# chengstone/cchess-zero

Measured on NVIDIA H100. Metric: mcts_node_expansions_per_sec, higher is better.
Workload: dtype fp16

## Files before the change

### cchess_zero_b200/_lib.py

```python
import ctypes as C
import os

_HERE = os.path.dirname(os.path.abspath(__file__))
LIB_PATH = os.path.join(_HERE, "libcchess_b200.so")

NSQ, NLABEL, MAXCHILD, ENC_LEN, STATUS_BYTES, MT_WORDS = 90, 2086, 128, 1260, 112, 626
F32, BF16, F16, BOARD = 0, 1, 2, 3
ERR_NAMES = {1: "NOMOVES", 2: "NOLABEL", 4: "DEPTH", 8: "ARENA", 16: "CHILDREN"}

_lib = None


class EngineError(RuntimeError):
    pass


def _sig(L):
    vp, i32, i64 = C.c_void_p, C.c_int, C.c_int64
    L.cz_last_error.restype = C.c_char_p
    L.cz_labels.argtypes = [vp]
    L.cz_label_index.argtypes = [i32, i32]
    L.cz_unflipped_index.argtypes = [vp]
    L.cz_from_state.argtypes = [C.c_char_p, vp]
    L.cz_to_state.argtypes = [vp, C.c_char_p]
# ... 21 lines not shown
    L.cz_engine_leaf_hashes.argtypes = [vp, vp]
    L.cz_engine_root_keys.argtypes = [vp, vp, vp]
    L.cz_engine_play_status.argtypes = [vp, vp, vp, vp]
    L.cz_engine_status_packed.argtypes = [vp, vp, vp]
    L.cz_engine_unfinished.argtypes = [vp, vp, vp]
    L.cz_engine_unfinished_async.argtypes = [vp, vp, vp]
    L.cz_engine_root_children.argtypes = [vp, vp, vp, vp, vp, vp, vp, vp]
    L.cz_engine_play.argtypes = [vp, vp, vp]
    L.cz_engine_status.argtypes = [vp, vp, vp, vp, vp, vp, vp, vp]
    L.cz_engine_counters.argtypes = [vp, vp, vp]
    L.cz_engine_tree_signature.argtypes = [vp, vp, i32, vp, i64, vp]
    L.cz_net_first_conv.argtypes = [vp, i32, vp, vp, vp, vp]
    L.cz_net_first_conv_tc.argtypes = [vp, i32, vp, vp, vp, vp]
    L.cz_net_first_conv_mma.argtypes = [vp, i32, vp, vp, vp]
    L.cz_net_heads.argtypes = [vp, i32, vp, vp, vp, vp, vp, vp, vp, vp, vp, vp, vp, vp, vp]
    L.cz_host_choose_moves.argtypes = [i32, vp, vp, vp, i32, vp, vp, vp, vp, i32]
    L.cz_net_heads_tc.argtypes = [vp, i32, vp, vp, vp, vp, vp, vp, vp, vp, vp, vp, vp, vp, vp]
    L.cz_net_heads_fc.argtypes = [vp, vp, i32, vp, vp, vp, vp, vp, vp, vp, vp, vp]
    L.cz_net_split_tf32.argtypes = [vp, vp, vp, i64, vp]
    L.cz_net_epilogue_split.argtypes = [vp, vp, vp, vp, vp, vp, vp, i64, vp]
    L.cz_net_tower_blob_bytes.argtypes = [i32]
    L.cz_net_tower_blob_bytes.restype = i64
    L.cz_net_tower_small.argtypes = [vp, i32, i32, i32, vp, vp, vp, vp, vp, vp, vp, vp]


def lib():
    global _lib
    if _lib is None:
        from . import build as _build

        distributed = "RANK" in os.environ or os.environ.get("CCHESS_NO_REBUILD", "0") == "1"
        if not (distributed and os.path.exists(LIB_PATH)):
            try:
                _build.build()
            except Exception as e:
                if not os.path.exists(LIB_PATH):
                    raise EngineError("libcchess_b200.so is missing and could not be built: %s" % e)
        L = C.CDLL(LIB_PATH)
        _sig(L)
        _lib = L
    return _lib


def check(rc, what=""):
    if rc != 0:
        raise EngineError("%s failed (%d): %s" % (what or "cchess_b200 call", rc, lib().cz_last_error().decode()))
# ... 1 lines not shown
```

### cchess_zero_b200/csrc/cz_net.cu

```cuda
#include <cuda_fp16.h>
#include <cuda_runtime.h>
#include <stdint.h>
#include <stdlib.h>
#include <string.h>

#include "../../include/cchess_b200.h"
#include "cz_wgmma.cuh"

namespace {

using namespace cz_sm90;

__global__ void __launch_bounds__(256) k_first_conv(const uint8_t *__restrict__ boards, int B, const __half *__restrict__ w ,
                                                     const float4 *__restrict__ bias , __half *__restrict__ out ) {
    __shared__ uint8_t pb[11 * 12 + 12];
    const int pos = blockIdx.x;
    const uint8_t *bd = boards + (size_t)pos * 96;
    if (threadIdx.x < 132) {
        const int r = threadIdx.x / 12 - 1, f = threadIdx.x % 12 - 1;
        pb[threadIdx.x] = (r >= 0 && r < 9 && f >= 0 && f < 10) ? bd[r * 9 + f] : (uint8_t)0;
    }
    __syncthreads();
    const int hw = threadIdx.x >> 4, l16 = threadIdx.x & 15;
    const float4 b0 = bias[l16 * 2], b1 = bias[l16 * 2 + 1];
// ... 3 lines not shown
        int pc[9];
#pragma unroll
        for (int t = 0; t < 9; t++) pc[t] = c0[(t / 3) * 12 + (t % 3)];
        float acc[8] = {b0.x, b0.y, b0.z, b0.w, b1.x, b1.y, b1.z, b1.w};
#pragma unroll
        for (int t = 0; t < 9; t++) {
            if (pc[t]) {
                const uint4 raw = __ldg(reinterpret_cast<const uint4 *>(w + ((size_t)(t * 14 + pc[t] - 1) * 128 + l16 * 8)));
                const __half2 *h2 = reinterpret_cast<const __half2 *>(&raw);
#pragma unroll
                for (int k = 0; k < 4; k++) {
                    const float2 v = __half22float2(h2[k]);
                    acc[2 * k] += v.x;
                    acc[2 * k + 1] += v.y;
                }
            }
        }
        uint4 o;
        __half2 *oh = reinterpret_cast<__half2 *>(&o);
#pragma unroll
        for (int k = 0; k < 4; k++) oh[k] = __floats2half2_rn(fmaxf(acc[2 * k], 0.f), fmaxf(acc[2 * k + 1], 0.f));
        *reinterpret_cast<uint4 *>(out + ((size_t)pos * 90 + cell) * 128 + l16 * 8) = o;
    }
}

__device__ __forceinline__ void mma16816(float (&c)[4], const uint32_t (&a)[4], const uint32_t (&b)[2]) {
    asm volatile("mma.sync.aligned.m16n8k16.row.col.f32.f16.f16.f32 {%0,%1,%2,%3}, {%4,%5,%6,%7}, {%8,%9}, {%0,%1,%2,%3};\n"
                 : "+f"(c[0]), "+f"(c[1]), "+f"(c[2]), "+f"(c[3])
                 : "r"(a[0]), "r"(a[1]), "r"(a[2]), "r"(a[3]), "r"(b[0]), "r"(b[1]));
}

constexpr int FCM_POS = 4;
__global__ void __launch_bounds__(256) k_first_conv_mma(const uint8_t *__restrict__ boards, int B, const uint2 *__restrict__ wfrag ,
                                                         __half *__restrict__ out ) {
    __shared__ uint2 sW[9 * 16 * 32];
    __shared__ uint8_t pb[FCM_POS][11 * 12 + 12];
    const int tid = threadIdx.x, warp = tid >> 5, lane = tid & 31, g = lane >> 2, t = lane & 3;
    const int pos0 = blockIdx.x * FCM_POS;
    for (int i = tid; i < 9 * 16 * 32 / 2; i += 256) reinterpret_cast<uint4 *>(sW)[i] = __ldg(reinterpret_cast<const uint4 *>(wfrag) + i);
    for (int i = tid; i < FCM_POS * 144; i += 256) {
        const int p = i / 144, j = i - p * 144;
        uint8_t v = 0;
        if (j < 132 && pos0 + p < B) {
            const int r = j / 12 - 1, f = j % 12 - 1;
            if (r >= 0 && r < 9 && f >= 0 && f < 10) v = boards[(size_t)(pos0 + p) * 96 + r * 9 + f];
        }
        pb[p][j] = v;
    }
    __syncthreads();
#pragma unroll 1
    for (int tile = warp; tile < FCM_POS * 6; tile += 8) {
        const int p = tile / 6, mt = tile - p * 6;
// ... 499 lines not shown
    if (cudaGetLastError() != cudaSuccess) return CZ_ECUDA;
    if (cudaEventRecord(ev_join[dev], side[dev]) != cudaSuccess) return CZ_ECUDA;
    dim3 grid((B + 63) / 64, NPAD / 64);
    k_policy_fc<<<grid, 128, smem, st>>>((const __half *)hp, B, (const __half *)wp, bp, logits);
    if (cudaGetLastError() != cudaSuccess) return CZ_ECUDA;
    if (cudaStreamWaitEvent(st, ev_join[dev], 0) != cudaSuccess) return CZ_ECUDA;
    return CZ_OK;
}

int cz_net_heads(const void *x, int B, const float *wh, const float *bh, const float *w1t, const float *b1, const float *w2, const float *b2,
                 const void *wp, const float *bp, void *hp_scratch, float *hv_scratch, float *logits, float *value, void *stream) {
    if (!x || !wh || !bh || !hp_scratch || !hv_scratch || B <= 0) return CZ_EINVAL;
    static const bool legacy = getenv("CCHESS_HEAD_CONV") && !strcmp(getenv("CCHESS_HEAD_CONV"), "simt");
    if (legacy) k_head_conv<<<B, 256, 0, (cudaStream_t)stream>>>((const __half *)x, B, wh, bh, (__half *)hp_scratch, hv_scratch);
    else k_head_conv_mma<false><<<B, 192, 0, (cudaStream_t)stream>>>((const __half *)x, B, wh, bh, (__half *)hp_scratch, hv_scratch);
    if (cudaGetLastError() != cudaSuccess) return CZ_ECUDA;
    return cz_net_heads_fc(hp_scratch, hv_scratch, B, w1t, b1, w2, b2, wp, bp, logits, value, stream);
}


int cz_net_heads_tc(const void *x, int B, const float *wh, const float *bh, const float *w1t, const float *b1, const float *w2, const float *b2,
                    const void *wp_tiled, const float *bp, void *hp_tiled_scratch, float *hv_scratch, float *logits, float *value, void *stream) {
    if (!x || !wh || !bh || !w1t || !b1 || !w2 || !b2 || !wp_tiled || !bp || !hp_tiled_scratch || !hv_scratch || !logits || !value || B <= 0) return CZ_EINVAL;
    cudaStream_t st = (cudaStream_t)stream;
    const int smem = 2 * FC_TILE_BYTES;
    if (cudaFuncSetAttribute(k_policy_fc_tc, cudaFuncAttributeMaxDynamicSharedMemorySize, smem) != cudaSuccess) return CZ_ECUDA;
    k_head_conv_mma<true><<<B, 192, 0, st>>>((const __half *)x, B, wh, bh, (__half *)hp_tiled_scratch, hv_scratch);
    if (cudaGetLastError() != cudaSuccess) return CZ_ECUDA;
    int dev = 0;
    if (cudaGetDevice(&dev) != cudaSuccess || dev < 0 || dev >= 64) return CZ_ECUDA;
    static cudaStream_t side[64] = {nullptr};
    static cudaEvent_t ev_fork[64] = {nullptr}, ev_join[64] = {nullptr};
    if (!side[dev]) {
        if (cudaStreamCreateWithFlags(&side[dev], cudaStreamNonBlocking) != cudaSuccess) return CZ_ECUDA;
        if (cudaEventCreateWithFlags(&ev_fork[dev], cudaEventDisableTiming) != cudaSuccess) return CZ_ECUDA;
        if (cudaEventCreateWithFlags(&ev_join[dev], cudaEventDisableTiming) != cudaSuccess) return CZ_ECUDA;
    }
    if (cudaEventRecord(ev_fork[dev], st) != cudaSuccess) return CZ_ECUDA;
    if (cudaStreamWaitEvent(side[dev], ev_fork[dev], 0) != cudaSuccess) return CZ_ECUDA;
    k_value_mlp<<<(B + VM_POS - 1) / VM_POS, 256, 0, side[dev]>>>(hv_scratch, B, w1t, b1, w2, b2, value);
    if (cudaGetLastError() != cudaSuccess) return CZ_ECUDA;
    if (cudaEventRecord(ev_join[dev], side[dev]) != cudaSuccess) return CZ_ECUDA;
    dim3 grid((B + 127) / 128, 17);
    k_policy_fc_tc<<<grid, 256, smem, st>>>((const uint4 *)hp_tiled_scratch, B, (const uint4 *)wp_tiled, bp, logits);
    if (cudaGetLastError() != cudaSuccess) return CZ_ECUDA;
    if (cudaStreamWaitEvent(st, ev_join[dev], 0) != cudaSuccess) return CZ_ECUDA;
    return CZ_OK;
}

int cz_net_split_tf32(const float *y, float *hi, void *x2, long long n_pix, void *stream) {
    if (!y || !hi || !x2 || n_pix <= 0) return CZ_EINVAL;
    const long long n8 = n_pix * 16;
    int dev = 0, sms = 132;
    if (cudaGetDevice(&dev) == cudaSuccess) cudaDeviceGetAttribute(&sms, cudaDevAttrMultiProcessorCount, dev);
    long long blocks = (n8 + 255) / 256;
    if (blocks > 8LL * sms) blocks = 8LL * sms;
    k_split_tf32<<<(unsigned)blocks, 256, 0, (cudaStream_t)stream>>>(reinterpret_cast<const float4 *>(y), reinterpret_cast<float4 *>(hi),
                                                                    reinterpret_cast<uint4 *>(x2), n8);
    return cudaGetLastError() == cudaSuccess ? CZ_OK : CZ_ECUDA;
}

int cz_net_epilogue_split(const float *t, const void *s, const float *bias, const float *skip, float *x, float *hi, void *x2, long long n_pix, void *stream) {
    if (!t || !bias || n_pix <= 0 || (!x && !hi) || ((hi == nullptr) != (x2 == nullptr))) return CZ_EINVAL;
    const long long n8 = n_pix * 16;
    int dev = 0, sms = 132;
    if (cudaGetDevice(&dev) == cudaSuccess) cudaDeviceGetAttribute(&sms, cudaDevAttrMultiProcessorCount, dev);
    long long blocks = (n8 + 255) / 256;
// ... 10 lines not shown
```

### cchess_zero_b200/csrc/cz_tower.cu

```cuda
#include <cuda.h>
#include <cuda_fp16.h>
#include <cuda_runtime.h>
#include <stdint.h>
#include <stdio.h>
#include <stdlib.h>
#include <string.h>

#include "../../include/cchess_b200.h"
#include "cz_wgmma.cuh"

namespace {

using namespace cz_sm90;

constexpr int ROWS = 152;
constexpr int P0 = 12;
constexpr int LBO_A = ROWS * 16;
constexpr int A_BYTES = 16 * LBO_A;
constexpr int NMATH = 256;
constexpr int NMATH_WARPS = NMATH / 32;
constexpr int NTHREADS = NMATH + 32;

__device__ __forceinline__ uint32_t img_off(int chunk, int row) { return (uint32_t)(chunk * LBO_A + row * 16); }

// ... 256 lines not shown
                float s0 = a.bh[0], s1 = a.bh[1], s2 = a.bh[2];
#pragma unroll 4
                for (int c8 = 0; c8 < 16; c8++) {
                    const uint4 raw = *reinterpret_cast<const uint4 *>(bufX + img_off(c8, P0 + j));
                    const __half2 *h2 = reinterpret_cast<const __half2 *>(&raw);
#pragma unroll
                    for (int k = 0; k < 4; k++) {
                        const float2 x = __half22float2(h2[k]);
                        const int c = c8 * 8 + 2 * k;
                        s0 += x.x * __ldg(a.wh + c) + x.y * __ldg(a.wh + c + 1);
                        s1 += x.x * __ldg(a.wh + 128 + c) + x.y * __ldg(a.wh + 128 + c + 1);
                        s2 += x.x * __ldg(a.wh + 256 + c) + x.y * __ldg(a.wh + 256 + c + 1);
                    }
                }
                const int ci = rr * 10 + ff;
                *reinterpret_cast<__half2 *>(a.hp + (size_t)pos * 192 + ci * 2) = __floats2half2_rn(fmaxf(s0, 0.f), fmaxf(s1, 0.f));
                a.hv[(size_t)pos * 96 + ci] = fmaxf(s2, 0.f);
            }
            if (rank == 0 && tid < 12) a.hp[(size_t)pos * 192 + 180 + tid] = __float2half(0.f);
        }
    }
    __syncthreads();
    if (CL > 1) cluster_sync_all();
}

typedef CUresult (*EncodeTiledFn)(CUtensorMap *, CUtensorMapDataType, cuuint32_t, void *, const cuuint64_t *, const cuuint64_t *, const cuuint32_t *,
                                  const cuuint32_t *, CUtensorMapInterleave, CUtensorMapSwizzle, CUtensorMapL2promotion, CUtensorMapFloatOOBfill);

EncodeTiledFn encode_tiled() {
    static EncodeTiledFn fn = nullptr;
    if (!fn) {
        void *p = nullptr;
        cudaDriverEntryPointQueryResult q;
        if (cudaGetDriverEntryPoint("cuTensorMapEncodeTiled", &p, cudaEnableDefault, &q) != cudaSuccess || q != cudaDriverEntryPointSuccess) return nullptr;
        fn = (EncodeTiledFn)p;
    }
    return fn;
}

template <int CL, bool ASYNC_ST>
int launch_tower(const CUtensorMap &map, const TowerArgs &a, cudaStream_t st) {
    constexpr int NC = 128 / CL, S = CL == 1 ? 4 : (CL == 2 ? 8 : 16);
    const int n_layers = 1 + a.n_conv;
    const size_t smem = 2 * (size_t)A_BYTES + (size_t)S * NC * 256 + (size_t)n_layers * NC * 4;
    if (cudaFuncSetAttribute(k_tower_small<CL, ASYNC_ST>, cudaFuncAttributeMaxDynamicSharedMemorySize, (int)smem) != cudaSuccess) return CZ_ECUDA;
    cudaLaunchConfig_t cfg = {};
// ... 44 lines not shown
    struct TraceDump {
        const TowerArgs &a; cudaStream_t st; long long *dev; int *calls;
        ~TraceDump() {
            if (!a.trace || ++*calls != 20) return;
            long long h[64 * 8];
            cudaStreamSynchronize(st);
            cudaMemcpy(h, dev, sizeof(h), cudaMemcpyDeviceToHost);
            fprintf(stderr, "tower trace (clock64 deltas): layer: in_ready->w_ready, ->mma_issued, ->mma_done, ->(same), ->stores_issued, ->next in_ready\n");
            for (int L = 0; L < a.n_conv; L++) {
                const long long *r = h + L * 8, nxt = L + 1 < a.n_conv ? h[(L + 1) * 8] : r[5];
                fprintf(stderr, "  L%02d: %6lld %6lld %6lld %6lld %6lld %6lld | layer %6lld\n", L, r[1] - r[0], r[2] - r[1], r[3] - r[2], r[4] - r[3], r[5] - r[4], nxt - r[5], nxt - r[0]);
            }
        }
    } dump{a, st, trace_dev, &trace_calls};
    static const bool generic_st = getenv("CCHESS_TOWER_ST") && !strcmp(getenv("CCHESS_TOWER_ST"), "generic");
    switch (cluster) {
        case 1: return generic_st ? launch_tower<1, false>(map, a, st) : launch_tower<1, true>(map, a, st);
        case 2: return generic_st ? launch_tower<2, false>(map, a, st) : launch_tower<2, true>(map, a, st);
        case 4: return generic_st ? launch_tower<4, false>(map, a, st) : launch_tower<4, true>(map, a, st);
        default: return generic_st ? launch_tower<8, false>(map, a, st) : launch_tower<8, true>(map, a, st);
    }
}

}
```

### cchess_zero_b200/csrc/cz_wgmma.cuh

```cuda
#pragma once
#include <stdint.h>

namespace cz_sm90 {

__device__ __forceinline__ uint32_t smem_u32(const void *p) { return (uint32_t)__cvta_generic_to_shared(p); }

__device__ __forceinline__ uint64_t gmma_desc(uint32_t smem_addr, uint32_t lbo_bytes) {
    return (uint64_t)((smem_addr >> 4) & 0x3FFFu) | ((uint64_t)((lbo_bytes >> 4) & 0x3FFFu) << 16) | ((uint64_t)(128u >> 4) << 32);
}

__device__ __forceinline__ void wgmma_fence() { asm volatile("wgmma.fence.sync.aligned;" ::: "memory"); }
__device__ __forceinline__ void wgmma_commit() { asm volatile("wgmma.commit_group.sync.aligned;" ::: "memory"); }
template <int N>
__device__ __forceinline__ void wgmma_wait() { asm volatile("wgmma.wait_group.sync.aligned %0;" ::"n"(N) : "memory"); }

template <int R>
__device__ __forceinline__ void fence_regs(float (&d)[R]) {
#pragma unroll
    for (int i = 0; i < R; i++) asm volatile("" : "+f"(d[i])::"memory");
}

template <int N>
struct Wgmma;
template <> struct Wgmma<16> {
    static __device__ __forceinline__ void mma(float (&d)[8], uint64_t da, uint64_t db, uint32_t scale_d) {
        asm volatile("{\n\t.reg .pred p;\n\tsetp.ne.b32 p, %10, 0;\n\t"
                     "wgmma.mma_async.sync.aligned.m64n16k16.f32.f16.f16 {"
                     "%0, %1, %2, %3, %4, %5, %6, %7"
                     "}, %8, %9, p, 1, 1, 0, 0;\n\t}"
                     : "+f"(d[0]), "+f"(d[1]), "+f"(d[2]), "+f"(d[3]), "+f"(d[4]), "+f"(d[5]), "+f"(d[6]), "+f"(d[7])
                     : "l"(da), "l"(db), "r"(scale_d));
    }
};
template <> struct Wgmma<32> {
    static __device__ __forceinline__ void mma(float (&d)[16], uint64_t da, uint64_t db, uint32_t scale_d) {
        asm volatile("{\n\t.reg .pred p;\n\tsetp.ne.b32 p, %18, 0;\n\t"
                     "wgmma.mma_async.sync.aligned.m64n32k16.f32.f16.f16 {"
                     "%0, %1, %2, %3, %4, %5, %6, %7, %8, %9, %10, %11, %12, %13, %14, %15"
                     "}, %16, %17, p, 1, 1, 0, 0;\n\t}"
                     : "+f"(d[0]), "+f"(d[1]), "+f"(d[2]), "+f"(d[3]), "+f"(d[4]), "+f"(d[5]), "+f"(d[6]), "+f"(d[7]),
                       "+f"(d[8]), "+f"(d[9]), "+f"(d[10]), "+f"(d[11]), "+f"(d[12]), "+f"(d[13]), "+f"(d[14]), "+f"(d[15])
                     : "l"(da), "l"(db), "r"(scale_d));
// ... 14 lines not shown
    }
};
template <> struct Wgmma<128> {
    static __device__ __forceinline__ void mma(float (&d)[64], uint64_t da, uint64_t db, uint32_t scale_d) {
        asm volatile("{\n\t.reg .pred p;\n\tsetp.ne.b32 p, %66, 0;\n\t"
                     "wgmma.mma_async.sync.aligned.m64n128k16.f32.f16.f16 {"
                     "%0, %1, %2, %3, %4, %5, %6, %7, %8, %9, %10, %11, %12, %13, %14, %15, "
                     "%16, %17, %18, %19, %20, %21, %22, %23, %24, %25, %26, %27, %28, %29, %30, %31, "
                     "%32, %33, %34, %35, %36, %37, %38, %39, %40, %41, %42, %43, %44, %45, %46, %47, "
                     "%48, %49, %50, %51, %52, %53, %54, %55, %56, %57, %58, %59, %60, %61, %62, %63"
                     "}, %64, %65, p, 1, 1, 0, 0;\n\t}"
                     : "+f"(d[0]), "+f"(d[1]), "+f"(d[2]), "+f"(d[3]), "+f"(d[4]), "+f"(d[5]), "+f"(d[6]), "+f"(d[7]),
                       "+f"(d[8]), "+f"(d[9]), "+f"(d[10]), "+f"(d[11]), "+f"(d[12]), "+f"(d[13]), "+f"(d[14]), "+f"(d[15]),
                       "+f"(d[16]), "+f"(d[17]), "+f"(d[18]), "+f"(d[19]), "+f"(d[20]), "+f"(d[21]), "+f"(d[22]), "+f"(d[23]),
                       "+f"(d[24]), "+f"(d[25]), "+f"(d[26]), "+f"(d[27]), "+f"(d[28]), "+f"(d[29]), "+f"(d[30]), "+f"(d[31]),
                       "+f"(d[32]), "+f"(d[33]), "+f"(d[34]), "+f"(d[35]), "+f"(d[36]), "+f"(d[37]), "+f"(d[38]), "+f"(d[39]),
                       "+f"(d[40]), "+f"(d[41]), "+f"(d[42]), "+f"(d[43]), "+f"(d[44]), "+f"(d[45]), "+f"(d[46]), "+f"(d[47]),
                       "+f"(d[48]), "+f"(d[49]), "+f"(d[50]), "+f"(d[51]), "+f"(d[52]), "+f"(d[53]), "+f"(d[54]), "+f"(d[55]),
                       "+f"(d[56]), "+f"(d[57]), "+f"(d[58]), "+f"(d[59]), "+f"(d[60]), "+f"(d[61]), "+f"(d[62]), "+f"(d[63])
                     : "l"(da), "l"(db), "r"(scale_d));
    }
};

}
```

### cchess_zero_b200/net.py

```python
import os

import numpy as np
import torch
import torch.nn as nn
import torch.nn.functional as F

NLABEL = 2086


class RefBatchNorm(nn.Module):

    def __init__(self, ch, eps=1e-5, decay=0.999, update_moving_stats=False):
        super().__init__()
        self.eps, self.decay, self.update = eps, decay, update_moving_stats
        self.register_buffer("running_mean", torch.zeros(ch))
        self.register_buffer("running_var", torch.ones(ch))

    def forward(self, x):
        if self.training:
            mean = x.mean(dim=(0, 2, 3))
            var = x.var(dim=(0, 2, 3), unbiased=False)
            if self.update:
                n = x.numel() / x.shape[1]
                with torch.no_grad():
# ... 420 lines not shown
            return True
        return False

    def make_input(self, B):
        return torch.zeros((B, 96), dtype=torch.uint8, device=self.hp.device)

    @torch.no_grad()
    def __call__(self, boards, logits_out, value_out):
        B = boards.shape[0]
        assert B <= self.max_batch and boards.dtype == torch.uint8 and logits_out.dtype == torch.float32
        assert self.blob.numel() * 2 == self._lib.cz_net_tower_blob_bytes(self.n_conv)
        st = self._C.c_void_p(torch.cuda.current_stream().cuda_stream)
        rc = self._lib.cz_net_tower_small(boards.data_ptr(), B, self.cluster, self.n_conv, self.w1.data_ptr(), self.blob.data_ptr(), self.bias.data_ptr(),
                                          self.wh.data_ptr(), self.bh.data_ptr(), self.hp.data_ptr(), self.hv.data_ptr(), st)
        if rc:
            raise RuntimeError("cz_net_tower_small failed (%d)" % rc)
        rc = self._lib.cz_net_heads_fc(self.hp.data_ptr(), self.hv.data_ptr(), B, self.w1t.data_ptr(), self.bv1.data_ptr(), self.w2.data_ptr(),
                                       self.b2t.data_ptr(), self.wp.data_ptr(), self.bp.data_ptr(), logits_out.data_ptr(), value_out.data_ptr(), st)
        if rc:
            raise RuntimeError("cz_net_heads_fc failed (%d)" % rc)
        return None


class _Tf32:
    def __init__(self, on):
        self.on = on

    def __enter__(self):
        self.prev = (torch.backends.cudnn.allow_tf32, torch.backends.cuda.matmul.allow_tf32)
        torch.backends.cudnn.allow_tf32 = self.on
        torch.backends.cuda.matmul.allow_tf32 = self.on

    def __exit__(self, *a):
        torch.backends.cudnn.allow_tf32, torch.backends.cuda.matmul.allow_tf32 = self.prev


def train_step_module(net, opt, x, pi, z, learning_rate, c_l2=1e-4, global_norm=100, group=None):
    import torch.distributed as dist
    net.train()
    for gp in opt.param_groups:
        gp["lr"] = float(learning_rate)
    logits, value = net(x)
    policy_loss = (-(pi * F.log_softmax(logits, dim=1)).sum(dim=1)).mean()
    value_loss = F.mse_loss(value, z)
    l2 = sum((p * p).sum() for p in net.parameters()) * (0.5 * c_l2)
    loss = value_loss + policy_loss + l2
# ... 31 lines not shown
        self.c_l2 = 0.0001
        self.momentum = 0.9
        self.global_norm = 100
        self.global_step = 0
        self.precision = precision or os.environ.get("CCHESS_NN_PRECISION", "fp16")
        if seed is not None:
            torch.manual_seed(seed)
        self.net = PolicyValueNet(res_block_nums, self.filters_size, update_moving_stats).to(self.device)
        self.net = self.net.to(memory_format=torch.channels_last)
        self.opt = torch.optim.SGD(self.net.parameters(), lr=1e-3, momentum=self.momentum, nesterov=True)
        self._plan = None
        self.weights_version = 0
        self.train_restore()

    def plan(self):
        if self._plan is None:
            self.net.eval()
            self._plan = make_plan(self.net, self.precision, owner=self)
        self._plan.refresh_if_stale()
        return self._plan

    def native_plan(self, max_batch, first_conv=None):
        self.net.eval()
        return NativePlan(self.net, max_batch, first_conv, owner=self)

    def small_plan(self, max_batch, cluster=None):
        self.net.eval()
        return SmallTowerPlan(self.net, max_batch, cluster, owner=self)

    @property
    def nn_dtype(self):
        return _DT[self.precision]

    def forward_device(self, nn_in, logits_out=None, value_out=None):
        return self.plan()(nn_in, logits_out, value_out)

    def forward(self, positions):
        x = torch.as_tensor(np.asarray(positions, dtype=np.float32)).reshape(-1, 9, 10, 14)
        x = x.to(self.device, non_blocking=True).to(self.nn_dtype)
        logits, value = self.plan()(x)
        return logits.cpu().numpy(), value.reshape(-1, 1).cpu().numpy()

    def train_step(self, positions, probs, winners, learning_rate):
        x = torch.as_tensor(np.asarray(positions, dtype=np.float32)).reshape(-1, 9, 10, 14).to(self.device)
        pi = torch.as_tensor(np.asarray(probs, dtype=np.float32)).to(self.device)
        z = torch.as_tensor(np.asarray(winners, dtype=np.float32)).reshape(-1, 1).to(self.device)
# ... 46 lines not shown
```

### include/cchess_b200.h

```cpp
#ifndef CCHESS_B200_H
#define CCHESS_B200_H
#include <stdint.h>

#ifdef __cplusplus
extern "C" {
#endif

#define CZ_OK 0
#define CZ_EINVAL (-1)
#define CZ_ECUDA (-2)
#define CZ_ENOMEM (-3)
#define CZ_EENGINE (-4)

#define CZ_NSQ 90
#define CZ_NLABEL 2086
#define CZ_MAXCHILD 128
#define CZ_ENC_LEN 1260

#define CZ_F32 0
#define CZ_BF16 1
#define CZ_F16 2
#define CZ_BOARD 3

#define CZ_ERR_NOMOVES 1
// ... 68 lines not shown
int cz_engine_tree_signature(cz_engine *e, void *stream, int game, int64_t *out, int64_t cap, int64_t *n);

int cz_net_first_conv(const uint8_t *canon_boards, int B, const void *w1, const float *b1, void *out, void *stream);
int cz_net_first_conv_tc(const uint8_t *canon_boards, int B, const void *w_umma, const float *b1, void *out, void *stream);
int cz_net_first_conv_mma(const uint8_t *canon_boards, int B, const void *w_frag, void *out, void *stream);
int cz_net_heads(const void *x, int B, const float *wh, const float *bh, const float *w1t, const float *b1, const float *w2, const float *b2,
                 const void *wp, const float *bp, void *hp_scratch, float *hv_scratch, float *logits, float *value, void *stream);

#define CZ_MT_WORDS 626
int cz_host_choose_moves(int n_games, const uint8_t *live, const int32_t *n_children, const double *ex , int exploration,
                         uint32_t *mt_states , int32_t *choice , double *probs , uint8_t *fallback ,
                         int n_threads);

int cz_net_heads_tc(const void *x, int B, const float *wh, const float *bh, const float *w1t, const float *b1, const float *w2, const float *b2,
                    const void *wp_tiled, const float *bp, void *hp_tiled_scratch, float *hv_scratch, float *logits, float *value, void *stream);

int cz_net_heads_fc(const void *hp, const float *hv, int B, const float *w1t, const float *b1, const float *w2, const float *b2,
                    const void *wp, const float *bp, float *logits, float *value, void *stream);

int64_t cz_net_tower_blob_bytes(int n_conv);
int cz_net_tower_small(const uint8_t *canon_boards, int n_pos, int cluster, int n_conv, const void *w1, const void *wblob, const float *bias,
                       const float *wh, const float *bh, void *hp, float *hv, void *stream);

int cz_net_split_tf32(const float *y, float *hi, void *x2, long long n_pix, void *stream);
int cz_net_epilogue_split(const float *t, const void *s, const float *bias, const float *skip, float *x, float *hi, void *x2, long long n_pix, void *stream);

#ifdef __cplusplus
}
#endif
#endif
```

Measured before the change: 926,900.

## Add fused persistent trunk kernel running first conv, residual tower, and head conv

Adds a persistent warp-specialized kernel that keeps each group of positions' activations in shared memory across every residual conv. Weights stream through a TMA/mbarrier ring and the convs run as WGMMA, with the first conv and the 1x1 head conv fused in at either end. It writes the policy features already tiled for the tensor-core policy FC and is used by default when max batch is at least 256. The aim is to remove per-layer kernel launches and global-memory round trips of activations, at the cost of a large and complex kernel whose occupancy is limited to one block per SM.

```diff
diff --git a/cchess_zero_b200/_lib.py b/cchess_zero_b200/_lib.py
--- a/cchess_zero_b200/_lib.py
+++ b/cchess_zero_b200/_lib.py
@@ -67,6 +67,8 @@
     L.cz_net_tower_blob_bytes.argtypes = [i32]
     L.cz_net_tower_blob_bytes.restype = i64
     L.cz_net_tower_small.argtypes = [vp, i32, i32, i32, vp, vp, vp, vp, vp, vp, vp, vp]
+    L.cz_net_trunk.argtypes = [vp, i32, i32, vp, vp, vp, vp, vp, vp, vp, vp]
+    L.cz_net_heads_fc_tc.argtypes = [vp, vp, i32, vp, vp, vp, vp, vp, vp, vp, vp, vp]
 
 
 def lib():
diff --git a/cchess_zero_b200/csrc/cz_net.cu b/cchess_zero_b200/csrc/cz_net.cu
--- a/cchess_zero_b200/csrc/cz_net.cu
+++ b/cchess_zero_b200/csrc/cz_net.cu
@@ -49,12 +49,6 @@
         for (int k = 0; k < 4; k++) oh[k] = __floats2half2_rn(fmaxf(acc[2 * k], 0.f), fmaxf(acc[2 * k + 1], 0.f));
         *reinterpret_cast<uint4 *>(out + ((size_t)pos * 90 + cell) * 128 + l16 * 8) = o;
     }
-}
-
-__device__ __forceinline__ void mma16816(float (&c)[4], const uint32_t (&a)[4], const uint32_t (&b)[2]) {
-    asm volatile("mma.sync.aligned.m16n8k16.row.col.f32.f16.f16.f32 {%0,%1,%2,%3}, {%4,%5,%6,%7}, {%8,%9}, {%0,%1,%2,%3};\n"
-                 : "+f"(c[0]), "+f"(c[1]), "+f"(c[2]), "+f"(c[3])
-                 : "r"(a[0]), "r"(a[1]), "r"(a[2]), "r"(a[3]), "r"(b[0]), "r"(b[1]));
 }
 
 constexpr int FCM_POS = 4;
@@ -600,11 +594,17 @@
 int cz_net_heads_tc(const void *x, int B, const float *wh, const float *bh, const float *w1t, const float *b1, const float *w2, const float *b2,
                     const void *wp_tiled, const float *bp, void *hp_tiled_scratch, float *hv_scratch, float *logits, float *value, void *stream) {
     if (!x || !wh || !bh || !w1t || !b1 || !w2 || !b2 || !wp_tiled || !bp || !hp_tiled_scratch || !hv_scratch || !logits || !value || B <= 0) return CZ_EINVAL;
+    k_head_conv_mma<true><<<B, 192, 0, (cudaStream_t)stream>>>((const __half *)x, B, wh, bh, (__half *)hp_tiled_scratch, hv_scratch);
+    if (cudaGetLastError() != cudaSuccess) return CZ_ECUDA;
+    return cz_net_heads_fc_tc(hp_tiled_scratch, hv_scratch, B, w1t, b1, w2, b2, wp_tiled, bp, logits, value, stream);
+}
+
+int cz_net_heads_fc_tc(const void *hp_tiled, const float *hv, int B, const float *w1t, const float *b1, const float *w2, const float *b2,
+                       const void *wp_tiled, const float *bp, float *logits, float *value, void *stream) {
+    if (!hp_tiled || !hv || !w1t || !b1 || !w2 || !b2 || !wp_tiled || !bp || !logits || !value || B <= 0) return CZ_EINVAL;
     cudaStream_t st = (cudaStream_t)stream;
     const int smem = 2 * FC_TILE_BYTES;
     if (cudaFuncSetAttribute(k_policy_fc_tc, cudaFuncAttributeMaxDynamicSharedMemorySize, smem) != cudaSuccess) return CZ_ECUDA;
-    k_head_conv_mma<true><<<B, 192, 0, st>>>((const __half *)x, B, wh, bh, (__half *)hp_tiled_scratch, hv_scratch);
-    if (cudaGetLastError() != cudaSuccess) return CZ_ECUDA;
     int dev = 0;
     if (cudaGetDevice(&dev) != cudaSuccess || dev < 0 || dev >= 64) return CZ_ECUDA;
     static cudaStream_t side[64] = {nullptr};
@@ -616,11 +616,11 @@
     }
     if (cudaEventRecord(ev_fork[dev], st) != cudaSuccess) return CZ_ECUDA;
     if (cudaStreamWaitEvent(side[dev], ev_fork[dev], 0) != cudaSuccess) return CZ_ECUDA;
-    k_value_mlp<<<(B + VM_POS - 1) / VM_POS, 256, 0, side[dev]>>>(hv_scratch, B, w1t, b1, w2, b2, value);
+    k_value_mlp<<<(B + VM_POS - 1) / VM_POS, 256, 0, side[dev]>>>(hv, B, w1t, b1, w2, b2, value);
     if (cudaGetLastError() != cudaSuccess) return CZ_ECUDA;
     if (cudaEventRecord(ev_join[dev], side[dev]) != cudaSuccess) return CZ_ECUDA;
     dim3 grid((B + 127) / 128, 17);
-    k_policy_fc_tc<<<grid, 256, smem, st>>>((const uint4 *)hp_tiled_scratch, B, (const uint4 *)wp_tiled, bp, logits);
+    k_policy_fc_tc<<<grid, 256, smem, st>>>((const uint4 *)hp_tiled, B, (const uint4 *)wp_tiled, bp, logits);
     if (cudaGetLastError() != cudaSuccess) return CZ_ECUDA;
     if (cudaStreamWaitEvent(st, ev_join[dev], 0) != cudaSuccess) return CZ_ECUDA;
     return CZ_OK;
diff --git a/cchess_zero_b200/csrc/cz_tower.cu b/cchess_zero_b200/csrc/cz_tower.cu
--- a/cchess_zero_b200/csrc/cz_tower.cu
+++ b/cchess_zero_b200/csrc/cz_tower.cu
@@ -302,6 +302,253 @@
     }
     __syncthreads();
     if (CL > 1) cluster_sync_all();
+}
+
+constexpr int TB_NMAX = 160;
+constexpr int TB_ROWS = P0 + 2 * TB_NMAX + 12;
+constexpr int TB_LBO = TB_ROWS * 16;
+constexpr int TB_IMG = 16 * TB_LBO;
+constexpr int TB_STAGE_CHUNKS = 4;
+constexpr int TB_STAGE = TB_STAGE_CHUNKS * 128 * 16;
+constexpr int TB_STAGES_PER_CONV = 9 * 16 / TB_STAGE_CHUNKS;
+constexpr int TB_S = 6;
+constexpr int TB_SMEM = 2 * TB_IMG + TB_S * TB_STAGE;
+static_assert(TB_SMEM + 2 * TB_S * 8 <= 227 * 1024, "k_tower_batch shared memory exceeds the sm_90 opt-in limit");
+static_assert(TB_STAGE == TB_STAGE_CHUNKS * 128 * 8 * 2, "expect_tx byte count = one stage of fp16 weights");
+
+struct TrunkArgs {
+    const uint8_t *boards;
+    const __half *w1;
+    const unsigned char *wblob;
+    const float *bias;
+    const float *wh;
+    const float *bh;
+    __half *hp_tiled;
+    float *hv;
+    int pos_begin;
+    int n_pos;
+    int n_conv;
+};
+__device__ __forceinline__ bool tb_cell(int r, int npos) {
+    const int p = r / 110, l = r - p * 110;
+    return p < npos && l < 99 && l % 11 < 10;
+}
+__device__ __forceinline__ void stmatrix_x4_trans(uint32_t addr, uint32_t r0, uint32_t r1, uint32_t r2, uint32_t r3) {
+    asm volatile("stmatrix.sync.aligned.m8n8.x4.trans.shared.b16 [%0], {%1, %2, %3, %4};" ::"r"(addr), "r"(r0), "r"(r1), "r"(r2), "r"(r3) : "memory");
+}
+__device__ __forceinline__ void ldmatrix_x4_trans(uint32_t addr, uint32_t (&r)[4]) {
+    asm volatile("ldmatrix.sync.aligned.m8n8.x4.trans.shared.b16 {%0, %1, %2, %3}, [%4];" : "=r"(r[0]), "=r"(r[1]), "=r"(r[2]), "=r"(r[3]) : "r"(addr) : "memory");
+}
+__device__ __forceinline__ uint32_t pack_relu(float a, float b, bool ca, bool cb) {
+    const __half2 h = __floats2half2_rn(ca ? fmaxf(a, 0.f) : 0.f, cb ? fmaxf(b, 0.f) : 0.f);
+    return *reinterpret_cast<const uint32_t *>(&h);
+}
+
+template <int NH>
+__device__ __forceinline__ void tb_convs(const TrunkArgs &a, uint32_t x, uint32_t y, uint32_t ring, uint64_t *full, uint64_t *empty,
+                                         int &stage, uint32_t &phase, int npos) {
+    const int tid = threadIdx.x, warp = tid >> 5, lane = tid & 31, wg = tid >> 7, q = lane & 3;
+    const int cq = wg * 64 + (warp & 3) * 16 + (lane >> 2);
+    const uint32_t lane_off = (uint32_t)((wg * 8 + (warp & 3) * 2 + ((lane >> 3) & 1)) * TB_LBO + (P0 + 8 * (lane >> 4) + (lane & 7)) * 16);
+    static_assert(NH / 2 <= 96, "three mask words");
+    uint32_t cellbits[3] = {0u, 0u, 0u};
+#pragma unroll 1
+    for (int i = 0; i < NH / 2; i++) {
+        const uint32_t bit = tb_cell(NH * (i / (NH / 4)) + 8 * ((i % (NH / 4)) / 2) + 2 * q + (i & 1), npos) ? 1u << (i & 31) : 0u;
+        if (i < 32) cellbits[0] |= bit;
+        else if (i < 64) cellbits[1] |= bit;
+        else cellbits[2] |= bit;
+    }
+    float d[2][NH / 2];
+    for (int L = 0; L < a.n_conv; L++) {
+        const uint32_t src = (L & 1) ? y : x;
+        int prev = 0;
+        for (int s = 0; s < TB_STAGES_PER_CONV; s++) {
+            mbar_wait(&full[stage], phase);
+            const int cg = s / 9, t = s % 9;
+            const int shift = (t / 3 - 1) * 11 + (t % 3 - 1);
+            const uint64_t da = gmma_desc(ring + (uint32_t)(stage * TB_STAGE + wg * 64 * 16), 128 * 16);
+            const uint64_t db = gmma_desc(src + (uint32_t)((P0 + shift) * 16 + cg * TB_STAGE_CHUNKS * TB_LBO), TB_LBO);
+            wgmma_fence();
+#pragma unroll
+            for (int kk = 0; kk < TB_STAGE_CHUNKS / 2; kk++) {
+                const uint32_t acc = (s | kk) ? 1u : 0u;
+                Wgmma<NH>::mma(d[0], da + (uint64_t)((kk * 2 * 128 * 16) >> 4), db + (uint64_t)((kk * 2 * TB_LBO) >> 4), acc);
+                Wgmma<NH>::mma(d[1], da + (uint64_t)((kk * 2 * 128 * 16) >> 4), db + (uint64_t)((kk * 2 * TB_LBO + NH * 16) >> 4), acc);
+            }
+            wgmma_commit();
+            if (s > 0) {
+                wgmma_wait<1>();
+                if (lane == 0) mbar_arrive(&empty[prev]);
+            }
+            prev = stage;
+            if (++stage == TB_S) { stage = 0; phase ^= 1u; }
+        }
+        wgmma_wait<0>();
+        fence_regs(d[0]);
+        fence_regs(d[1]);
+        if (lane == 0) mbar_arrive(&empty[prev]);
+        const bool second = L & 1;
+        const uint32_t dst = second ? x : y;
+        const float b0 = __ldg(a.bias + (1 + L) * 128 + cq), b1 = __ldg(a.bias + (1 + L) * 128 + cq + 8);
+#pragma unroll
+        for (int h = 0; h < 2; h++) {
+#pragma unroll
+            for (int j = 0; j < NH / 8; j += 2) {
+                const uint32_t addr = dst + lane_off + (uint32_t)((NH * h + 8 * j) * 16);
+                uint32_t sk[4] = {0u, 0u, 0u, 0u};
+                if (second) ldmatrix_x4_trans(addr, sk);
+                uint32_t o[4];
+#pragma unroll
+                for (int m = 0; m < 4; m++) {
+                    const int jj = j + (m >> 1), ch = m & 1;
+                    const int i = (h * (NH / 8) + jj) * 2;
+                    float f0 = d[h][4 * jj + 2 * ch], f1 = d[h][4 * jj + 2 * ch + 1];
+                    if (second) {
+                        const float2 sv = __half22float2(*reinterpret_cast<const __half2 *>(&sk[m]));
+                        f0 += sv.x; f1 += sv.y;
+                    }
+                    f0 += ch ? b1 : b0; f1 += ch ? b1 : b0;
+                    o[m] = pack_relu(f0, f1, (cellbits[i / 32] >> (i % 32)) & 1u, (cellbits[(i + 1) / 32] >> ((i + 1) % 32)) & 1u);
+                }
+                stmatrix_x4_trans(addr, o[0], o[1], o[2], o[3]);
+            }
+        }
+        asm volatile("fence.proxy.async;" ::: "memory");
+        math_sync();
+    }
+}
+
+constexpr int TB_THREADS = NMATH + 128;
+
+template <int NH>
+__global__ void __launch_bounds__(TB_THREADS, 1) k_tower_batch(const __grid_constant__ TrunkArgs a) {
+    constexpr int P = NH == TB_NMAX ? 3 : 2;
+    static_assert(P * 110 - 11 <= 2 * NH, "a task's raster fits the MMA rows");
+    extern __shared__ __align__(128) unsigned char smem[];
+    __shared__ __align__(8) uint64_t full[TB_S], empty[TB_S];
+    const int tid = threadIdx.x, warp = tid >> 5, lane = tid & 31;
+    const uint32_t x = smem_u32(smem), y = x + TB_IMG, ring = x + 2 * TB_IMG;
+    const int n_tasks = (a.n_pos + P - 1) / P;
+
+    for (int i = tid; i < 2 * TB_IMG / 16; i += TB_THREADS) reinterpret_cast<uint4 *>(smem)[i] = make_uint4(0, 0, 0, 0);
+    if (tid == 0) {
+        for (int s = 0; s < TB_S; s++) { mbar_init(&full[s], 1); mbar_init(&empty[s], NMATH_WARPS); }
+        asm volatile("fence.mbarrier_init.release.cluster;" ::: "memory");
+    }
+    asm volatile("fence.proxy.async;" ::: "memory");
+    __syncthreads();
+
+    if (warp >= NMATH_WARPS) {
+        asm volatile("setmaxnreg.dec.sync.aligned.u32 40;");
+        if (warp == NMATH_WARPS && lane == 0) {
+            int stage = 0;
+            uint32_t phase = 0;
+            for (int task = blockIdx.x; task < n_tasks; task += gridDim.x)
+                for (int i = 0; i < a.n_conv * TB_STAGES_PER_CONV; i++) {
+                    mbar_wait(&empty[stage], phase ^ 1u);
+                    mbar_expect_tx(&full[stage], TB_STAGE);
+                    asm volatile("cp.async.bulk.shared::cluster.global.mbarrier::complete_tx::bytes [%0], [%1], %2, [%3];"
+                                 ::"r"(ring + (uint32_t)(stage * TB_STAGE)), "l"(a.wblob + (size_t)i * TB_STAGE), "r"(TB_STAGE),
+                                   "r"(smem_u32(&full[stage])) : "memory");
+                    if (++stage == TB_S) { stage = 0; phase ^= 1u; }
+                }
+        }
+        return;
+    }
+    asm volatile("setmaxnreg.inc.sync.aligned.u32 232;");
+    int stage = 0;
+    uint32_t phase = 0;
+    for (int task = blockIdx.x; task < n_tasks; task += gridDim.x) {
+        const int pos0 = a.pos_begin + task * P, npos = min(P, a.n_pos - task * P);
+        for (int it = tid; it < 2 * NH * 4; it += NMATH) {
+            const int r = it % (2 * NH), cq = it / (2 * NH);
+            const int p = r / 110, l = r - p * 110, rr = l / 11, ff = l - rr * 11;
+            const bool cell = p < npos && rr < 9 && ff < 10;
+            float acc[32];
+#pragma unroll
+            for (int c = 0; c < 32; c++) acc[c] = __ldg(a.bias + cq * 32 + c);
+            if (cell) {
+                const uint8_t *bd = a.boards + (size_t)(pos0 + p) * 96;
+#pragma unroll 1
+                for (int t = 0; t < 9; t++) {
+                    const int r2 = rr + t / 3 - 1, f2 = ff + t % 3 - 1;
+                    if (r2 < 0 || r2 >= 9 || f2 < 0 || f2 >= 10) continue;
+                    const int pc = __ldg(bd + r2 * 9 + f2);
+                    if (!pc) continue;
+                    const uint4 *wr = reinterpret_cast<const uint4 *>(a.w1 + (size_t)(t * 14 + pc - 1) * 128 + cq * 32);
+#pragma unroll
+                    for (int c8 = 0; c8 < 4; c8++) {
+                        const uint4 raw = __ldg(wr + c8);
+                        const __half2 *h2 = reinterpret_cast<const __half2 *>(&raw);
+#pragma unroll
+                        for (int k = 0; k < 4; k++) {
+                            const float2 v = __half22float2(h2[k]);
+                            acc[c8 * 8 + 2 * k] += v.x;
+                            acc[c8 * 8 + 2 * k + 1] += v.y;
+                        }
+                    }
+                }
+            }
+#pragma unroll
+            for (int c8 = 0; c8 < 4; c8++) {
+                uint4 o;
+                o.x = pack_relu(acc[c8 * 8 + 0], acc[c8 * 8 + 1], cell, cell);
+                o.y = pack_relu(acc[c8 * 8 + 2], acc[c8 * 8 + 3], cell, cell);
+                o.z = pack_relu(acc[c8 * 8 + 4], acc[c8 * 8 + 5], cell, cell);
+                o.w = pack_relu(acc[c8 * 8 + 6], acc[c8 * 8 + 7], cell, cell);
+                *reinterpret_cast<uint4 *>(smem + (cq * 4 + c8) * TB_LBO + (P0 + r) * 16) = o;
+            }
+        }
+        asm volatile("fence.proxy.async;" ::: "memory");
+        math_sync();
+        tb_convs<NH>(a, x, y, ring, full, empty, stage, phase, npos);
+        {
+            const int g = lane >> 2, t = lane & 3;
+            uint32_t bhi[8][2], blo[8][2];
+#pragma unroll
+            for (int ks = 0; ks < 8; ks++)
+#pragma unroll
+                for (int h = 0; h < 2; h++) {
+                    const int k = ks * 16 + h * 8 + t * 2;
+                    const float w0 = g < 3 ? __ldg(a.wh + g * 128 + k) : 0.f, w1 = g < 3 ? __ldg(a.wh + g * 128 + k + 1) : 0.f;
+                    const __half h0 = __float2half_rn(w0), h1 = __float2half_rn(w1);
+                    const __half l0 = __float2half_rn(w0 - __half2float(h0)), l1 = __float2half_rn(w1 - __half2float(h1));
+                    __half2 hh = __halves2half2(h0, h1), ll = __halves2half2(l0, l1);
+                    bhi[ks][h] = *reinterpret_cast<uint32_t *>(&hh);
+                    blo[ks][h] = *reinterpret_cast<uint32_t *>(&ll);
+                }
+            const float bh0 = __ldg(a.bh), bh1 = __ldg(a.bh + 1), bh2 = __ldg(a.bh + 2);
+            for (int row0 = warp * 16; row0 < npos * 110; row0 += NMATH_WARPS * 16) {
+                const int lr = min(row0 + (lane & 15), 2 * NH + 11);
+                const uint32_t abase = x + (uint32_t)((lane >> 4) * TB_LBO + (P0 + lr) * 16);
+                float acc[4] = {0.f, 0.f, 0.f, 0.f};
+#pragma unroll
+                for (int ks = 0; ks < 8; ks++) {
+                    uint32_t af[4];
+                    asm volatile("ldmatrix.sync.aligned.m8n8.x4.shared.b16 {%0, %1, %2, %3}, [%4];"
+                                 : "=r"(af[0]), "=r"(af[1]), "=r"(af[2]), "=r"(af[3]) : "r"(abase + (uint32_t)(ks * 2 * TB_LBO)));
+                    mma16816(acc, af, bhi[ks]);
+                    mma16816(acc, af, blo[ks]);
+                }
+#pragma unroll
+                for (int hlf = 0; hlf < 2; hlf++) {
+                    const int r = row0 + g + hlf * 8, p = r / 110, l = r - p * 110, rr = l / 11, ff = l - rr * 11;
+                    if (p >= npos || rr >= 9 || ff >= 10) continue;
+                    const int pos = pos0 + p, k = (rr * 10 + ff) * 2;
+                    if (t == 0)
+                        *reinterpret_cast<__half2 *>(a.hp_tiled + ((size_t)(pos >> 7) * 24 + (k >> 3)) * 1024 + (size_t)(pos & 127) * 8 + (k & 7)) =
+                            __floats2half2_rn(fmaxf(acc[hlf * 2] + bh0, 0.f), fmaxf(acc[hlf * 2 + 1] + bh1, 0.f));
+                    if (t == 1) a.hv[(size_t)pos * 96 + k / 2] = fmaxf(acc[hlf * 2] + bh2, 0.f);
+                }
+            }
+        }
+        for (int i = tid; i < npos * 12; i += NMATH) {
+            const int pos = pos0 + i / 12, k = 180 + i % 12;
+            a.hp_tiled[((size_t)(pos >> 7) * 24 + (k >> 3)) * 1024 + (size_t)(pos & 127) * 8 + (k & 7)] = __float2half(0.f);
+        }
+        math_sync();
+    }
 }
 
 typedef CUresult (*EncodeTiledFn)(CUtensorMap *, CUtensorMapDataType, cuuint32_t, void *, const cuuint64_t *, const cuuint64_t *, const cuuint32_t *,
@@ -392,4 +639,35 @@
     }
 }
 
-}
+int cz_net_trunk(const uint8_t *canon_boards, int n_pos, int n_conv, const void *w1, const void *wblob, const float *bias, const float *wh,
+                 const float *bh, void *hp_tiled, float *hv, void *stream) {
+    if (!canon_boards || !w1 || !wblob || !bias || !wh || !bh || !hp_tiled || !hv || n_pos <= 0 || n_conv <= 0 || (n_conv & 1)) return CZ_EINVAL;
+    if (((uintptr_t)wblob & 15) || ((uintptr_t)w1 & 15)) return CZ_EINVAL;
+    int dev = 0, sms = 132, optin = 0;
+    if (cudaGetDevice(&dev) != cudaSuccess) return CZ_ECUDA;
+    cudaDeviceGetAttribute(&sms, cudaDevAttrMultiProcessorCount, dev);
+    if (cudaDeviceGetAttribute(&optin, cudaDevAttrMaxSharedMemoryPerBlockOptin, dev) != cudaSuccess || optin < TB_SMEM + 2 * TB_S * 8) return CZ_ECUDA;
+    if (cudaFuncSetAttribute(k_tower_batch<TB_NMAX>, cudaFuncAttributeMaxDynamicSharedMemorySize, TB_SMEM) != cudaSuccess) return CZ_ECUDA;
+    if (cudaFuncSetAttribute(k_tower_batch<112>, cudaFuncAttributeMaxDynamicSharedMemorySize, TB_SMEM) != cudaSuccess) return CZ_ECUDA;
+    TrunkArgs a;
+    a.boards = canon_boards; a.w1 = (const __half *)w1; a.wblob = (const unsigned char *)wblob; a.bias = bias; a.wh = wh; a.bh = bh;
+    a.hp_tiled = (__half *)hp_tiled; a.hv = hv; a.n_conv = n_conv;
+    cudaStream_t st = (cudaStream_t)stream;
+    const long long round3 = 3LL * sms, rem = n_pos % round3;
+    const int n3 = rem > 2LL * sms ? n_pos : (int)(n_pos - rem);
+    if (n3 > 0) {
+        a.pos_begin = 0; a.n_pos = n3;
+        const int tasks = (n3 + 2) / 3;
+        k_tower_batch<TB_NMAX><<<tasks < sms ? tasks : sms, TB_THREADS, TB_SMEM, st>>>(a);
+        if (cudaGetLastError() != cudaSuccess) return CZ_ECUDA;
+    }
+    if (n3 < n_pos) {
+        a.pos_begin = n3; a.n_pos = n_pos - n3;
+        const int tasks = (a.n_pos + 1) / 2;
+        k_tower_batch<112><<<tasks, TB_THREADS, TB_SMEM, st>>>(a);
+        if (cudaGetLastError() != cudaSuccess) return CZ_ECUDA;
+    }
+    return CZ_OK;
+}
+
+}
diff --git a/cchess_zero_b200/csrc/cz_wgmma.cuh b/cchess_zero_b200/csrc/cz_wgmma.cuh
--- a/cchess_zero_b200/csrc/cz_wgmma.cuh
+++ b/cchess_zero_b200/csrc/cz_wgmma.cuh
@@ -18,6 +18,12 @@
 __device__ __forceinline__ void fence_regs(float (&d)[R]) {
 #pragma unroll
     for (int i = 0; i < R; i++) asm volatile("" : "+f"(d[i])::"memory");
+}
+
+__device__ __forceinline__ void mma16816(float (&c)[4], const uint32_t (&a)[4], const uint32_t (&b)[2]) {
+    asm volatile("mma.sync.aligned.m16n8k16.row.col.f32.f16.f16.f32 {%0,%1,%2,%3}, {%4,%5,%6,%7}, {%8,%9}, {%0,%1,%2,%3};\n"
+                 : "+f"(c[0]), "+f"(c[1]), "+f"(c[2]), "+f"(c[3])
+                 : "r"(a[0]), "r"(a[1]), "r"(a[2]), "r"(a[3]), "r"(b[0]), "r"(b[1]));
 }
 
 template <int N>
@@ -78,4 +84,47 @@
     }
 };
 
+template <> struct Wgmma<112> {
+    static __device__ __forceinline__ void mma(float (&d)[56], uint64_t da, uint64_t db, uint32_t scale_d) {
+        asm volatile("{\n\t.reg .pred p;\n\tsetp.ne.b32 p, %58, 0;\n\t"
+                     "wgmma.mma_async.sync.aligned.m64n112k16.f32.f16.f16 {"
+                     "%0, %1, %2, %3, %4, %5, %6, %7, %8, %9, %10, %11, %12, %13, %14, %15, "
+                     "%16, %17, %18, %19, %20, %21, %22, %23, %24, %25, %26, %27, %28, %29, %30, %31, "
+                     "%32, %33, %34, %35, %36, %37, %38, %39, %40, %41, %42, %43, %44, %45, %46, %47, "
+                     "%48, %49, %50, %51, %52, %53, %54, %55"
+                     "}, %56, %57, p, 1, 1, 0, 0;\n\t}"
+                     : "+f"(d[0]), "+f"(d[1]), "+f"(d[2]), "+f"(d[3]), "+f"(d[4]), "+f"(d[5]), "+f"(d[6]), "+f"(d[7]),
+                       "+f"(d[8]), "+f"(d[9]), "+f"(d[10]), "+f"(d[11]), "+f"(d[12]), "+f"(d[13]), "+f"(d[14]), "+f"(d[15]),
+                       "+f"(d[16]), "+f"(d[17]), "+f"(d[18]), "+f"(d[19]), "+f"(d[20]), "+f"(d[21]), "+f"(d[22]), "+f"(d[23]),
+                       "+f"(d[24]), "+f"(d[25]), "+f"(d[26]), "+f"(d[27]), "+f"(d[28]), "+f"(d[29]), "+f"(d[30]), "+f"(d[31]),
+                       "+f"(d[32]), "+f"(d[33]), "+f"(d[34]), "+f"(d[35]), "+f"(d[36]), "+f"(d[37]), "+f"(d[38]), "+f"(d[39]),
+                       "+f"(d[40]), "+f"(d[41]), "+f"(d[42]), "+f"(d[43]), "+f"(d[44]), "+f"(d[45]), "+f"(d[46]), "+f"(d[47]),
+                       "+f"(d[48]), "+f"(d[49]), "+f"(d[50]), "+f"(d[51]), "+f"(d[52]), "+f"(d[53]), "+f"(d[54]), "+f"(d[55])
+                     : "l"(da), "l"(db), "r"(scale_d));
+    }
+};
+template <> struct Wgmma<160> {
+    static __device__ __forceinline__ void mma(float (&d)[80], uint64_t da, uint64_t db, uint32_t scale_d) {
+        asm volatile("{\n\t.reg .pred p;\n\tsetp.ne.b32 p, %82, 0;\n\t"
+                     "wgmma.mma_async.sync.aligned.m64n160k16.f32.f16.f16 {"
+                     "%0, %1, %2, %3, %4, %5, %6, %7, %8, %9, %10, %11, %12, %13, %14, %15, "
+                     "%16, %17, %18, %19, %20, %21, %22, %23, %24, %25, %26, %27, %28, %29, %30, %31, "
+                     "%32, %33, %34, %35, %36, %37, %38, %39, %40, %41, %42, %43, %44, %45, %46, %47, "
+                     "%48, %49, %50, %51, %52, %53, %54, %55, %56, %57, %58, %59, %60, %61, %62, %63, "
+                     "%64, %65, %66, %67, %68, %69, %70, %71, %72, %73, %74, %75, %76, %77, %78, %79"
+                     "}, %80, %81, p, 1, 1, 0, 0;\n\t}"
+                     : "+f"(d[0]), "+f"(d[1]), "+f"(d[2]), "+f"(d[3]), "+f"(d[4]), "+f"(d[5]), "+f"(d[6]), "+f"(d[7]),
+                       "+f"(d[8]), "+f"(d[9]), "+f"(d[10]), "+f"(d[11]), "+f"(d[12]), "+f"(d[13]), "+f"(d[14]), "+f"(d[15]),
+                       "+f"(d[16]), "+f"(d[17]), "+f"(d[18]), "+f"(d[19]), "+f"(d[20]), "+f"(d[21]), "+f"(d[22]), "+f"(d[23]),
+                       "+f"(d[24]), "+f"(d[25]), "+f"(d[26]), "+f"(d[27]), "+f"(d[28]), "+f"(d[29]), "+f"(d[30]), "+f"(d[31]),
+                       "+f"(d[32]), "+f"(d[33]), "+f"(d[34]), "+f"(d[35]), "+f"(d[36]), "+f"(d[37]), "+f"(d[38]), "+f"(d[39]),
+                       "+f"(d[40]), "+f"(d[41]), "+f"(d[42]), "+f"(d[43]), "+f"(d[44]), "+f"(d[45]), "+f"(d[46]), "+f"(d[47]),
+                       "+f"(d[48]), "+f"(d[49]), "+f"(d[50]), "+f"(d[51]), "+f"(d[52]), "+f"(d[53]), "+f"(d[54]), "+f"(d[55]),
+                       "+f"(d[56]), "+f"(d[57]), "+f"(d[58]), "+f"(d[59]), "+f"(d[60]), "+f"(d[61]), "+f"(d[62]), "+f"(d[63]),
+                       "+f"(d[64]), "+f"(d[65]), "+f"(d[66]), "+f"(d[67]), "+f"(d[68]), "+f"(d[69]), "+f"(d[70]), "+f"(d[71]),
+                       "+f"(d[72]), "+f"(d[73]), "+f"(d[74]), "+f"(d[75]), "+f"(d[76]), "+f"(d[77]), "+f"(d[78]), "+f"(d[79])
+                     : "l"(da), "l"(db), "r"(scale_d));
+    }
+};
+
 }
diff --git a/cchess_zero_b200/net.py b/cchess_zero_b200/net.py
--- a/cchess_zero_b200/net.py
+++ b/cchess_zero_b200/net.py
@@ -466,6 +466,92 @@
         return None
 
 
+class TrunkPlan:
+
+    precision = "fp16"
+    dtype = torch.uint8
+    first_conv = "trunk"
+
+    def __init__(self, net, max_batch, owner=None):
+        import ctypes as C
+        from ._lib import lib
+        self._C, self._lib = C, lib()
+        self._base = InferencePlan(net, "fp16", owner=owner)
+        self.fused = True
+        self.net, self.owner, self.version = net, owner, self._base.version
+        self.n_conv = 2 * len(self._base.blocks)
+        assert self.n_conv > 0
+        for k, v in self._derive().items():
+            setattr(self, k, v)
+        dev = self._base.w_in[0].device
+        self.max_batch = max_batch
+        self.hv = torch.zeros((max_batch, 96), dtype=torch.float32, device=dev)
+        self.hp_tiled = torch.zeros(((max_batch + 127) // 128, 24, 128, 8), dtype=torch.float16, device=dev)
+
+    def _derive(self):
+        net, base = self.net, self._base
+        dev = base.w_in[0].device
+        with torch.no_grad():
+            w, b = base.w_in
+            w1 = w.float().permute(2, 3, 1, 0).reshape(9, 14, 128).to(torch.float16).contiguous()
+            convs = [c for blk in base.blocks for c in blk]
+            bias = torch.stack([b.float()] + [cb.float() for _, cb in convs]).contiguous()
+            blob = torch.stack([cw.permute(2, 3, 0, 1).reshape(9, 128, 4, 4, 8).permute(2, 0, 3, 1, 4) for cw, _ in convs]).to(torch.float16).contiguous()
+            wh, bh = base.w_head
+            wp_pad = torch.zeros((2176, 192), dtype=torch.float16, device=dev)
+            wp_pad[:NLABEL, :180] = net.p_fc.weight.detach().to(torch.float16)
+            bp_pad = torch.zeros((2176,), dtype=torch.float32, device=dev)
+            bp_pad[:NLABEL] = net.p_fc.bias.detach().float()
+            return dict(w1=w1, bias=bias, blob=blob, wh=wh.float().reshape(3, 128).contiguous(), bh=bh.float().contiguous(),
+                        w1t=net.v_fc1.weight.detach().float().t().contiguous(), bv1=net.v_fc1.bias.detach().float().contiguous(),
+                        w2=net.v_fc2.weight.detach().float().reshape(256).contiguous(),
+                        b2t=net.v_fc2.bias.detach().float().reshape(1).contiguous(),
+                        wp_tiled=wp_pad.reshape(17, 128, 24, 8).permute(0, 2, 1, 3).contiguous(), bp_pad=bp_pad)
+
+    def refresh(self):
+        self._base.refresh()
+        with torch.no_grad():
+            for k, v in self._derive().items():
+                getattr(self, k).copy_(v)
+        self.version = self._base.version
+
+    def refresh_if_stale(self):
+        if self.owner is not None and self.owner.weights_version != self.version:
+            self.refresh()
+            return True
+        return False
+
+    def make_input(self, B):
+        return torch.zeros((B, 96), dtype=torch.uint8, device=self.hv.device)
+
+    def trunk(self, boards):
+        B = boards.shape[0]
+        assert B <= self.max_batch and boards.dtype == torch.uint8 and boards.is_contiguous()
+        assert self.blob.numel() * 2 == self._lib.cz_net_tower_blob_bytes(self.n_conv)
+        rc = self._lib.cz_net_trunk(boards.data_ptr(), B, self.n_conv, self.w1.data_ptr(), self.blob.data_ptr(), self.bias.data_ptr(),
+                                    self.wh.data_ptr(), self.bh.data_ptr(), self.hp_tiled.data_ptr(), self.hv.data_ptr(),
+                                    self._C.c_void_p(torch.cuda.current_stream().cuda_stream))
+        if rc:
+            raise RuntimeError("cz_net_trunk failed (%d)" % rc)
+
+    def heads(self, B, logits_out, value_out):
+        assert logits_out.dtype == torch.float32
+        rc = self._lib.cz_net_heads_fc_tc(self.hp_tiled.data_ptr(), self.hv.data_ptr(), B, self.w1t.data_ptr(), self.bv1.data_ptr(),
+                                          self.w2.data_ptr(), self.b2t.data_ptr(), self.wp_tiled.data_ptr(), self.bp_pad.data_ptr(),
+                                          logits_out.data_ptr(), value_out.data_ptr(), self._C.c_void_p(torch.cuda.current_stream().cuda_stream))
+        if rc:
+            raise RuntimeError("cz_net_heads_fc_tc failed (%d)" % rc)
+
+    @torch.no_grad()
+    def __call__(self, boards, logits_out, value_out):
+        self.trunk(boards)
+        self.heads(boards.shape[0], logits_out, value_out)
+        return None
+
+
+TRUNK_MIN_BATCH = 256
+
+
 class _Tf32:
     def __init__(self, on):
         self.on = on
@@ -543,6 +629,8 @@
 
     def native_plan(self, max_batch, first_conv=None):
         self.net.eval()
+        if first_conv is None and "CCHESS_FIRST_CONV" not in os.environ and max_batch >= TRUNK_MIN_BATCH and len(self.net.blocks) > 0:
+            return TrunkPlan(self.net, max_batch, owner=self)
         return NativePlan(self.net, max_batch, first_conv, owner=self)
 
     def small_plan(self, max_batch, cluster=None):
diff --git a/include/cchess_b200.h b/include/cchess_b200.h
--- a/include/cchess_b200.h
+++ b/include/cchess_b200.h
@@ -114,6 +114,11 @@
 int cz_net_tower_small(const uint8_t *canon_boards, int n_pos, int cluster, int n_conv, const void *w1, const void *wblob, const float *bias,
                        const float *wh, const float *bh, void *hp, float *hv, void *stream);
 
+int cz_net_trunk(const uint8_t *canon_boards, int n_pos, int n_conv, const void *w1, const void *wblob, const float *bias, const float *wh,
+                 const float *bh, void *hp_tiled, float *hv, void *stream);
+int cz_net_heads_fc_tc(const void *hp_tiled, const float *hv, int B, const float *w1t, const float *b1, const float *w2, const float *b2,
+                       const void *wp_tiled, const float *bp, float *logits, float *value, void *stream);
+
 int cz_net_split_tf32(const float *y, float *hi, void *x2, long long n_pix, void *stream);
 int cz_net_epilogue_split(const float *t, const void *s, const float *bias, const float *skip, float *x, float *hi, void *x2, long long n_pix, void *stream);
 
```

Result: faster. 1.063 million (median of 6 runs) (+14.7%).
